# mosaicml/streaming

Measured on AMD Instinct MI355X. Metric: decoded samples/sec + MDS GiB/s, device-resident, at 1/2/4/8 MI355X, higher is better.
Workload: dtype u8

## Files before the change

### streaming_amd/csrc/mdsx_decode.h

```cpp
#pragma once

#include <hip/hip_runtime.h>

#include <cstdint>

#include "mdsx_device.h"
#include "mdsx_internal.h"

namespace mdsx_kernels {

constexpr int kBlock = 256;
constexpr int kSmallMax = 16;
constexpr uint64_t kMapGrain = uint64_t(kBlock) * 16;
constexpr int kGatherRows = 1024;
constexpr int kGroupUnroll = 2;

struct DevCol {
  void* data;
  int64_t* offsets;
  uint8_t* flags;
  uint64_t capacity;
  uint32_t row_bytes;
  int8_t kind;
  int8_t var_index;
  int8_t gather;
  int8_t group;
};

struct TileRun {
  uint64_t stream;
  uint64_t offs;
  uint64_t row0;
  uint32_t bytes;
  uint32_t shard;
  uint32_t r0;
  uint16_t nrows;
  uint16_t fast;
  uint64_t shard_off;
};
static_assert(sizeof(TileRun) == 48, "TileRun layout");

constexpr uint32_t kXcdSeg = 1, kXcdRegister = 2, kXcdRows = 4;

struct DevArgs {
  const uint8_t* batch;
  const mdsx_shard_desc* shards;
  const uint32_t* tile_shard;
  mdsx_status* status;
  int64_t* tile_total;
  int64_t* tile_prefix;
  int64_t* chunk_sum;
  TileRun* tile_run;
  int64_t* totals;
  uint64_t* src_abs;
  uint32_t* row_map;
  uint64_t* lookback;
  uint32_t* ticket;
  uint64_t map_len;
  uint64_t rows;
  uint32_t ntiles;
  uint32_t nscan;
  uint32_t nchunk;
  uint32_t scan_per;
  int32_t nshards;
  int32_t ncols;
  int32_t nvar;
  int32_t tile_rows;
  int16_t any_group;
  int16_t any_wave_str;
  int16_t any_wave_ragged;
  int16_t str_cached;
  uint32_t stage_debug;
  uint32_t run_slots;
  uint32_t rows_bytes;
  uint32_t seg_lim;
  uint32_t seg_small;
  uint32_t xcd_order;
  uint32_t rows_pipe;
  uint32_t rw_k;
  uint32_t swave;
  uint4* sw_rec;
  uint32_t sw_lds;
  uint32_t gather_block0[MDSX_MAX_COLUMNS + 1];
  DevCol cols[MDSX_MAX_COLUMNS];
};


constexpr uint32_t kSwIdle = 0xffffffffu, kSwBad = 0xfffffffeu;

struct TileView {
  const uint8_t* shard;
  const uint32_t* offs;
  mdsx_shard_desc d;
  uint32_t shard_idx;
  uint32_t r0;
  uint32_t nrows;
  uint64_t hdr_end;
  bool table_ok;
};

__device__ __forceinline__ uint32_t xcd_block(uint32_t b, uint32_t n) {
  const uint32_t per = n >> 3;
  return b < per * 8u ? (b & 7u) * per + (b >> 3) : b;
}

__device__ __forceinline__ TileView tile_view(const DevArgs& a, uint32_t tile) {
  TileView v;
  v.shard_idx = a.tile_shard[tile];
  v.d = a.shards[v.shard_idx];
  v.shard = a.batch + v.d.offset;
  v.offs = reinterpret_cast<const uint32_t*>(v.shard + 4);
  v.r0 = (tile - v.d.tile0) * uint32_t(a.tile_rows);
  v.nrows = v.d.samples > v.r0 ? min(uint32_t(a.tile_rows), v.d.samples - v.r0) : 0u;
  v.hdr_end = 4ull + 4ull * (uint64_t(v.d.samples) + 1ull);
  v.table_ok = v.hdr_end <= v.d.bytes;
  return v;
}

__device__ __forceinline__ int sample_range(const TileView& v, uint32_t i, uint32_t* b,
                                            uint32_t* e) {
  *b = v.offs[i];
  *e = v.offs[i + 1];
  if (!(v.hdr_end <= *b && *b <= *e && *e <= v.d.bytes)) return MDSX_E_BOUNDS;
  if (*b == *e) return MDSX_E_EMPTY;
  return MDSX_OK;
}

__device__ __forceinline__ void lds_barrier() {
  asm volatile("s_waitcnt lgkmcnt(0)\n\ts_barrier" ::: "memory");
}

template <bool kRaw = false>
__device__ __forceinline__ int64_t block_exclusive_scan(int64_t x, int64_t* s_wsum,
                                                        int64_t* total) {
  const int lane = threadIdx.x & 63, w = threadIdx.x >> 6;
  int64_t incl = x;
#pragma unroll
  for (int o = 1; o < 64; o <<= 1) {
    const int64_t y = __shfl_up(incl, o);
    if (lane >= o) incl += y;
  }
  if (lane == 63) s_wsum[w] = incl;
  if constexpr (kRaw) lds_barrier();
  else __syncthreads();
  int64_t base = 0, tot = 0;
#pragma unroll
  for (int k = 0; k < kBlock / 64; ++k) {
    const int64_t s = s_wsum[k];
    base += (k < w) ? s : 0;
    tot += s;
  }
  if constexpr (kRaw) lds_barrier();
  else __syncthreads();
  *total = tot;
  return base + incl - x;
}


constexpr uint64_t kHugeCountOffset = 192;
constexpr uint64_t kErrKindsOffset = 64;
constexpr uint32_t kRowLevelErrors = (1u << -MDSX_E_BOUNDS) | (1u << -MDSX_E_EMPTY);

__device__ __forceinline__ void report_decode(const DevArgs& a, int code, int shard, int row,
                                              int col) {
  report(a.status, code, shard, row, col);
  atomicOr(reinterpret_cast<uint32_t*>(reinterpret_cast<uint8_t*>(a.status) + kErrKindsOffset),
           1u << ((-code) & 31));
}

constexpr uint64_t kStatusBlock = 256;

constexpr uint64_t kLbAggregate = 1ull << 62, kLbInclusive = 2ull << 62;
constexpr uint64_t kLbValue = (1ull << 62) - 1;
typedef __attribute__((address_space(1))) uint64_t gu64;

__device__ __forceinline__ void lookback_bases(const DevArgs& a, uint32_t tile, const int64_t* agg,
                                               int64_t* base_out, uint32_t shard, int lane,
                                               uint64_t* words, uint32_t nunits) {
  const int nv = a.nvar;
  const int W = nv <= 1 ? 64 : nv <= 2 ? 32 : nv <= 4 ? 16 : 8;
  const int kk = lane & (W - 1);
  const int seg0 = lane & ~(W - 1);
  const uint64_t wmask = W == 64 ? ~0ull : (1ull << W) - 1;
  for (int g0 = 0; g0 < nv; g0 += 64 / W) {
    const int vi = g0 + lane / W;
    const bool mine = vi < nv;
    gu64* st = (gu64*)(words + uint64_t(mine ? vi : 0) * nunits);
    const uint64_t ag = mine ? uint64_t(agg[vi]) : 0;
    if (mine && kk == 0)
      __hip_atomic_store(st + tile, (tile == 0 ? kLbInclusive : kLbAggregate) | ag,
                         __ATOMIC_RELAXED, __HIP_MEMORY_SCOPE_AGENT);
    uint64_t base = 0;
    int64_t j = int64_t(tile) - 1;
    bool done = !mine || tile == 0;
    uint32_t polls = 0;
    while (__ballot(!done) != 0) {
      const int64_t k = j - kk;
      const uint64_t w = (!done && k >= 0) ? __hip_atomic_load(st + k, __ATOMIC_RELAXED,
                                                               __HIP_MEMORY_SCOPE_AGENT)
                                           : kLbInclusive;
      const uint64_t incl = (__ballot((w >> 62) == 2) >> seg0) & wmask;
      const uint64_t none = (__ballot((w >> 62) == 0) >> seg0) & wmask;
      const uint64_t span = incl ? ((incl & (0 - incl)) << 1) - 1 : wmask;
      const bool wait = !done && (none & span) != 0 && ++polls < (1u << 22);
      uint64_t x = (!done && !wait && ((span >> kk) & 1)) ? (w & kLbValue) : 0;
      for (int o = W >> 1; o > 0; o >>= 1) x += __shfl_xor(x, o);
      if (!done && !wait) {
        if ((none & span) != 0 && kk == 0) report_decode(a, MDSX_E_HIP, int(shard), -1, -1);
        base += x;
        if (incl) done = true;
        else j -= W;
      }
      if (__ballot(wait) != 0) __builtin_amdgcn_s_sleep(1);
    }
    if (mine && kk == 0) {
      if (tile != 0)
        __hip_atomic_store(st + tile, kLbInclusive | (base + ag), __ATOMIC_RELAXED,
                           __HIP_MEMORY_SCOPE_AGENT);
      base_out[vi] = int64_t(base);
      if (tile + 1 == nunits) {
        for (int c = 0; c < a.ncols; ++c)
          if (a.cols[c].var_index == vi) a.cols[c].offsets[a.rows] = int64_t(base + ag);
        if (a.totals) a.totals[vi] = int64_t(base + ag);
      }
    }
  }
}

__device__ __forceinline__ uint32_t draw_ticket(const DevArgs& a, uint32_t* s_tile) {
  if (threadIdx.x == 0) *s_tile = atomicAdd(a.ticket, 1u);
  __syncthreads();
  return __builtin_amdgcn_readfirstlane(*s_tile);
}

int launch_stage_totals(const DevArgs& a, bool nt, hipStream_t s);
int launch_run_decode(const mdsx_plan* plan, const DevArgs& a, hipStream_t s);
int launch_rows_decode(const mdsx_plan* plan, const DevArgs& a, hipStream_t s);
int launch_huge_rows(const DevArgs& a, bool nt, hipStream_t s);
int launch_swave_decode(const mdsx_plan* plan, const DevArgs& a, hipStream_t s);

}
```

### streaming_amd/csrc/mdsx_kernels.hip

```cpp
#include <hip/hip_runtime.h>

#include <algorithm>
#include <cstdint>
#include <cstring>

#include "mdsx_decode.h"
#include "mdsx_device.h"
#include "mdsx_internal.h"

namespace mdsx_kernels {

template <bool kRec = false>
__global__ __launch_bounds__(kBlock) void scan_tiles_kernel(const DevArgs a) {
  __shared__ int64_t s_wsum[kBlock / 64];
  const int t = threadIdx.x;
  const int TR = a.tile_rows;
  const int per_block = kBlock / TR;
  const uint32_t tile = blockIdx.x * uint32_t(per_block) + uint32_t(t / TR);
  const int tt = t % TR;
  const bool tile_ok = tile < a.ntiles;
  TileView v;
  if (tile_ok) v = tile_view(a, tile);
  const uint32_t i = tile_ok ? v.r0 + tt : 0;
  const bool in_tile = tile_ok && v.table_ok && tt < int(v.nrows);
// ... 443 lines not shown
  const int64_t* off;
  const uint64_t* src;
  __device__ __forceinline__ int64_t o(int i) const { return off[i]; }
  __device__ __forceinline__ uint64_t s(int i) const { return src[i]; }
};

template <class Rows>
__device__ __forceinline__ int find_row(const Rows& R, int n, int64_t D) {
  int lo = 0, hi = n - 1;
  while (lo < hi) {
    const int mid = (lo + hi + 1) >> 1;
    if (R.o(mid) <= D) lo = mid; else hi = mid - 1;
  }
  return lo;
}

template <bool kNT, class Rows>
__device__ __forceinline__ uint4 assemble(const Rows& R, int n, int j, int64_t D,
                                          const uint8_t* batch) {
  uint4 acc = make_uint4(0, 0, 0, 0);
  for (; j < n && R.o(j) < D + 16; ++j) {
    const int64_t ro = R.o(j), re = R.o(j + 1);
    const int64_t a = max(D, ro), b = min(D + 16, re);
    if (b <= a) continue;
    const uint64_t s0 = reinterpret_cast<uint64_t>(batch) + R.s(j) + uint64_t(D - ro);
    const uint4* al = reinterpret_cast<const uint4*>(s0 & ~uint64_t(15));
    const uint32_t sh = uint32_t(s0 & 15);
    const uint4 lo = ld16<kNT>(al);
    const uint4 hi = sh ? ld16<kNT>(al + 1) : make_uint4(0, 0, 0, 0);
    const uint4 val = sh ? funnel16_lane(lo, hi, sh) : lo;
    const uint4 m = byte_mask(uint32_t(a - D), uint32_t(b - D));
    acc = make_uint4((acc.x & ~m.x) | (val.x & m.x), (acc.y & ~m.y) | (val.y & m.y),
                     (acc.z & ~m.z) | (val.z & m.z), (acc.w & ~m.w) | (val.w & m.w));
  }
  return acc;
}

template <class Rows>
__device__ __forceinline__ void utf8_check(const Rows& R, int n, int j, int64_t D, int64_t tot,
                                           const uint4 v, uint32_t pw, uint8_t* flags,
                                           uint64_t row0) {
  uint32_t p1 = (pw >> 24) & 0xffu, p2 = (pw >> 16) & 0xffu, p3 = (pw >> 8) & 0xffu;
  const bool ascii = ((v.x | v.y | v.z | v.w) & 0x80808080u) == 0;
  if (ascii && p1 < 0xC0u && p2 < 0xE0u && p3 < 0xF0u) return;
  const int64_t dist = D - R.o(j);
  if (dist < 3) p3 = 0;
  if (dist < 2) p2 = 0;
  if (dist < 1) p1 = 0;
  int64_t rend = R.o(j + 1);
  bool bad = false;
#pragma unroll
  for (int k = 0; k < 16; ++k) {
    const int64_t P = D + k;
    if (P >= tot) break;
    if (P >= rend) {
      if (bad) flags[row0 + j] = 1;
      bad = false;
      do {
        ++j;
        rend = R.o(j + 1);
      } while (P >= rend && j + 1 < n);
      p1 = p2 = p3 = 0;
    }
    const uint32_t b = byte_of(v, k);
    const bool cont = (b & 0xC0u) == 0x80u;
    const bool need = p1 >= 0xC0u || p2 >= 0xE0u || p3 >= 0xF0u;
    const int64_t left = rend - P;
    bad |= cont != need;
    bad |= b == 0xC0u || b == 0xC1u || b >= 0xF5u;
    bad |= (p1 == 0xE0u && b < 0xA0u) || (p1 == 0xEDu && b > 0x9Fu) ||
           (p1 == 0xF0u && b < 0x90u) || (p1 == 0xF4u && b > 0x8Fu);
    bad |= (b >= 0xC0u && left <= 1) || (b >= 0xE0u && left <= 2) || (b >= 0xF0u && left <= 3);
    p3 = p2;
    p2 = p1;
    p1 = b;
  }
  if (bad) flags[row0 + j] = 1;
}

template <bool kNT, int kGatherChunks, class Rows>
__device__ __forceinline__ void gather_tile(const DevArgs& a, const DevCol& col, const Rows& R,
                                            int n, uint64_t r0, int64_t T0, int64_t tot,
                                            uint32_t* s_edge) {
  const bool utf8 = col.kind == MDSX_KIND_STR && col.flags;
  uint8_t* out = static_cast<uint8_t*>(col.data);
  const int lane = threadIdx.x & 63, wave = threadIdx.x >> 6;
  const uint64_t base = reinterpret_cast<uint64_t>(a.batch);
  uint4 val[kGatherChunks], lo[kGatherChunks], hi[kGatherChunks];
  int jrow[kGatherChunks];
  uint32_t shift[kGatherChunks];
  bool single[kGatherChunks], need_hi[kGatherChunks];
#pragma unroll
  for (int k = 0; k < kGatherChunks; ++k) {
    const int64_t D = T0 + 16 * (threadIdx.x + kBlock * k);
    const bool valid = D < tot;
    const int j = valid ? find_row(R, n, D) : 0;
    const int64_t ro = R.o(j), re = R.o(j + 1);
    const uint64_t s0 = base + R.s(j) + uint64_t(D - ro);
    const uint4* al = reinterpret_cast<const uint4*>(s0 & ~uint64_t(15));
    jrow[k] = j;
    shift[k] = uint32_t(s0 & 15);
    single[k] = valid && D + 16 <= re;
    const bool next_same = single[k] && D + 16 < re && lane != 63;
    need_hi[k] = single[k] && shift[k] != 0 && !next_same;
    lo[k] = valid ? ld16<kNT>(al) : make_uint4(0, 0, 0, 0);
    hi[k] = need_hi[k] ? ld16<kNT>(al + 1) : make_uint4(0, 0, 0, 0);
  }
#pragma unroll
  for (int k = 0; k < kGatherChunks; ++k) {
    const int64_t D = T0 + 16 * (threadIdx.x + kBlock * k);
    const uint4 nb = shfl_down1(lo[k]);
    if (single[k]) {
      const uint4 h = need_hi[k] ? hi[k] : nb;
      val[k] = shift[k] ? funnel16_lane(lo[k], h, shift[k]) : lo[k];
    } else if (D < tot) {
      val[k] = assemble<kNT>(R, n, jrow[k], D, a.batch);
    } else {
      val[k] = make_uint4(0, 0, 0, 0);
    }
    if (D < tot) {
      const uint64_t dst = reinterpret_cast<uint64_t>(out) + uint64_t(D);
      if (uint64_t(D) + 16 <= col.capacity) {
        st16<kNT>(dst, val[k]);
      } else {
        for (int b = 0; b < 16 && uint64_t(D) + b < col.capacity; ++b)
          out[D + b] = uint8_t(byte_of(val[k], b));
      }
    }
  }
  if (!utf8) return;
#pragma unroll
  for (int k = 0; k < kGatherChunks; ++k)
    if (lane == 63) s_edge[k * (kBlock / 64) + wave] = val[k].w;
  __syncthreads();
#pragma unroll
  for (int k = 0; k < kGatherChunks; ++k) {
    const int c = threadIdx.x + kBlock * k;
    const int64_t D = T0 + 16 * c;
    uint32_t pw = __shfl_up(val[k].w, 1);
    if (lane == 0) {
      if (c == 0)
        pw = D > R.o(0) ? assemble<kNT>(R, 1, 0, D - 16, a.batch).w : 0u;
      else
        pw = s_edge[wave > 0 ? k * (kBlock / 64) + wave - 1 : (k - 1) * (kBlock / 64) + 3];
    }
    if (D < tot) utf8_check(R, n, jrow[k], D, tot, val[k], pw, col.flags, r0);
  }
}

template <bool kNT, int kGatherChunks>
__global__ __launch_bounds__(kBlock) void gather_ragged_kernel(const DevArgs a) {
  constexpr uint64_t kGatherTile = kMapGrain * kGatherChunks;
  __shared__ __attribute__((aligned(16))) int64_t s_off[kGatherRows + 1];
  __shared__ uint64_t s_src[kGatherRows];
  __shared__ uint32_t s_edge[kGatherChunks * (kBlock / 64)];
  int vi = 0;
  while (vi + 1 < a.nvar && blockIdx.x >= a.gather_block0[vi + 1]) ++vi;
  int ci = 0;
  while (a.cols[ci].var_index != vi) ++ci;
  const DevCol& col = a.cols[ci];
  const int64_t tot = col.offsets[a.rows];
  const uint32_t kinds =
      *reinterpret_cast<const uint32_t*>(reinterpret_cast<const uint8_t*>(a.status) + kErrKindsOffset);
  if (kinds & ~kRowLevelErrors) return;
  const uint32_t* map = a.row_map + uint64_t(vi) * a.map_len;
  const uint64_t* src = a.src_abs + uint64_t(vi) * a.rows;
  const uint64_t stride = a.gather_block0[vi + 1] - a.gather_block0[vi];
  for (uint64_t g = blockIdx.x - a.gather_block0[vi];; g += stride) {
    const int64_t T0 = int64_t(g * kGatherTile);
    if (T0 >= tot || (g + 1) * kGatherChunks >= a.map_len) return;
    const uint64_t r0 = map[g * kGatherChunks];
    const uint64_t r1 =
        (T0 + int64_t(kGatherTile) < tot) ? uint64_t(map[(g + 1) * kGatherChunks]) : a.rows - 1;
    if (r0 >= a.rows || r1 >= a.rows || r1 < r0) return;
    const int n = int(r1 - r0 + 1);
    __syncthreads();
    if (n <= kGatherRows) {
      for (int i = threadIdx.x; i <= n; i += kBlock) {
        s_off[i] = col.offsets[r0 + i];
        if (i < n) s_src[i] = src[r0 + i];
      }
      __syncthreads();
      gather_tile<kNT, kGatherChunks>(a, col, RowsLds{s_off, s_src}, n, r0, T0, tot, s_edge);
    } else {
      gather_tile<kNT, kGatherChunks>(a, col, RowsGlobal{col.offsets + r0, src + r0}, n, r0,
                                      T0, tot, s_edge);
    }
  }
}

struct Layout {
  uint64_t tile_total, tile_prefix, chunk_sum, tile_run, src_abs, row_map, sw_rec, map_len,
      total;
};

__host__ uint64_t round256(uint64_t x) { return (x + 255) & ~uint64_t(255); }

constexpr uint64_t kTicketOffset = 128;

Layout workspace_layout(const mdsx_plan* plan, const mdsx_batch* b) {
  Layout L;
  const uint64_t nv = uint64_t(plan->nvar);
  L.map_len = b->bytes / kMapGrain + 8;
  L.tile_total = 256;
  L.tile_prefix = L.tile_total + round256(nv * b->ntiles * 8);
  L.chunk_sum = L.tile_prefix + round256(nv * b->ntiles * 8);
  L.tile_run = L.chunk_sum + round256(nv * (b->ntiles / kScanChunk + 1) * 8);
  L.src_abs = L.tile_run + round256(nv ? uint64_t(b->ntiles) * sizeof(TileRun) : 0);
  L.row_map = L.src_abs + round256(nv * b->rows * 8);
  L.sw_rec = L.row_map + round256(nv * L.map_len * 4);
  L.total = L.sw_rec + round256(use_swave_decode(plan, b->bytes, b->rows)
                                    ? uint64_t(b->ntiles) *
                                          uint64_t(b->tile_rows ? b->tile_rows
                                                                : uint32_t(plan->tile_rows)) * 16
                                    : 0);
  return L;
}

int build_args(const mdsx_plan* plan, const mdsx_batch* b, const mdsx_column_out* outs,
               void* d_workspace, uint64_t workspace_bytes, int64_t* d_totals, DevArgs* a,
               const uint64_t* mode_bytes = nullptr) {
  if (!plan || !b || !b->data || !b->shards || !b->tile_shard || !d_workspace ||
      b->nshards <= 0)
    return mdsx::fail(MDSX_E_ARG, "mdsx: null argument or empty batch");
  if (plan->ncols > 0 && !outs) return mdsx::fail(MDSX_E_ARG, "mdsx: outs is NULL");
  const Layout L = workspace_layout(plan, b);
  if (workspace_bytes < L.total)
    return mdsx::fail(MDSX_E_ARG, "mdsx: workspace smaller than mdsx_workspace_bytes()");
  std::memset(a, 0, sizeof(*a));
  a->batch = b->data;
  a->shards = b->shards;
  a->tile_shard = b->tile_shard;
  uint8_t* ws = static_cast<uint8_t*>(d_workspace);
  a->status = reinterpret_cast<mdsx_status*>(ws);
  a->tile_total = reinterpret_cast<int64_t*>(ws + L.tile_total);
  a->tile_prefix = reinterpret_cast<int64_t*>(ws + L.tile_prefix);
  a->chunk_sum = reinterpret_cast<int64_t*>(ws + L.chunk_sum);
  a->tile_run = reinterpret_cast<TileRun*>(ws + L.tile_run);
  a->src_abs = reinterpret_cast<uint64_t*>(ws + L.src_abs);
  a->row_map = reinterpret_cast<uint32_t*>(ws + L.row_map);
  a->sw_rec = reinterpret_cast<uint4*>(ws + L.sw_rec);
  a->lookback = reinterpret_cast<uint64_t*>(ws + L.tile_total);
  a->ticket = reinterpret_cast<uint32_t*>(ws + kTicketOffset);
  a->map_len = L.map_len;
  a->totals = d_totals;
  a->rows = b->rows;
  a->ntiles = b->ntiles;
  const int tr = b->tile_rows ? int(b->tile_rows) : plan->tile_rows;
  if (tr < 1 || tr > kBlock || (tr & (tr - 1)))
    return mdsx::fail(MDSX_E_ARG, "mdsx: batch tile_rows must be a power of two in [1, 256]");
  a->stage_debug = uint32_t(plan->stage_debug);
  a->xcd_order = uint32_t(plan->xcd_order);
  a->rw_k = uint32_t(plan->rowwave_k);
  a->swave = use_swave_decode(plan, b->bytes, b->rows) ? 1u : 0u;
  a->run_slots = use_run_decode(plan, b->bytes, b->rows) && !a->swave ? uint32_t(plan->run_slots)
                                                                      : 0u;
  if (a->run_slots && plan->seg) {
    a->seg_lim = a->run_slots * 1024u - 1024u - 32u;
    for (int c = 0; c < plan->ncols; ++c)
      if (plan->cols[c].kind == MDSX_KIND_FIXED && plan->cols[c].row_bytes <= kSmallMax)
        a->seg_small += uint32_t(plan->cols[c].row_bytes);
  }
  a->rows_bytes = use_rows_decode(plan, b->bytes, b->rows)
                      ? rows_stage_bytes(plan, b->bytes / b->rows, tr)
                      : 0u;
  if (a->rows_bytes && rows_lds_bytes_est(plan, a->rows_bytes, uint64_t(tr)) > 160 * 1024)
    a->rows_bytes = 0;
  a->rows_pipe = a->rows_bytes ? uint32_t(plan->rows_pipe) : 0u;
  if (a->run_slots && tr > 32)
    return mdsx::fail(MDSX_E_ARG, "mdsx: streaming decode tiles hold at most 32 rows");
  a->scan_per = (a->run_slots || a->rows_bytes) ? 1u : uint32_t(kBlock / tr);
  a->nscan = (b->ntiles + a->scan_per - 1) / a->scan_per;
  a->nchunk = (a->nscan + kScanChunk - 1) / kScanChunk;
  a->nshards = b->nshards;
  a->ncols = plan->ncols;
  a->nvar = plan->nvar;
  a->tile_rows = tr;
  uint32_t gblocks = 0;
  const uint64_t tile = kMapGrain * uint64_t(plan->gather_chunks);
  for (int c = 0; c < plan->ncols; ++c) {
    const mdsx::ColumnSpec& s = plan->cols[c];
    DevCol& d = a->cols[c];
    d.data = outs[c].data;
    d.offsets = outs[c].offsets;
    d.flags = outs[c].flags;
    d.capacity = outs[c].capacity;
    d.row_bytes = uint32_t(s.row_bytes);
    d.kind = int8_t(s.kind);
    d.var_index = int8_t(s.var_index);
    const uint64_t expect =
        mode_bytes ? std::min(mode_bytes[c], outs[c].capacity) : outs[c].capacity;
    d.gather = s.kind != MDSX_KIND_FIXED && b->rows > 0 &&
               expect < uint64_t(plan->gather_min) * b->rows;
    d.group = s.kind != MDSX_KIND_FIXED && !d.gather && b->rows > 0 &&
              expect < uint64_t(plan->group_max) * b->rows;
    if (s.kind == MDSX_KIND_FIXED) {
      if (!d.data && b->rows > 0)
        return mdsx::fail(MDSX_E_ARG, "mdsx: null data pointer for a fixed column");
    } else {
      if (!d.offsets || (!d.data && d.capacity > 0))
        return mdsx::fail(MDSX_E_ARG, "mdsx: null offsets/data for a ragged column");
    }
  }
  for (int c = 0; c < plan->ncols; ++c) {
    const DevCol& d = a->cols[c];
    if (d.group) a->any_group = 1;
    if (d.kind != MDSX_KIND_FIXED && !d.gather && !d.group) a->any_wave_ragged = 1;
    if (d.kind == MDSX_KIND_STR && d.flags && !d.gather) a->any_wave_str = 1;
    a->str_cached = int16_t(plan->str_cached);
  }
  for (int v = 0; v < plan->nvar; ++v) {
    a->gather_block0[v] = gblocks;
    for (int c = 0; c < plan->ncols; ++c)
      if (plan->cols[c].var_index == v && a->cols[c].gather) {
        const uint64_t expect =
            mode_bytes ? std::min(mode_bytes[c], outs[c].capacity) : outs[c].capacity;
        gblocks += uint32_t(expect > tile ? (expect + tile - 1) / tile : 1);
      }
  }
  a->gather_block0[plan->nvar] = gblocks;
  return MDSX_OK;
}

int hip_check(hipError_t e, const char* what) {
  if (e == hipSuccess) return MDSX_OK;
  return mdsx::fail(MDSX_E_HIP, std::string(what) + ": " + hipGetErrorString(e));
}

constexpr uint64_t kProbeBlock = 256 * 1024 / 16;
__global__ __launch_bounds__(kBlock) void copy_probe_kernel(const uint4* __restrict__ src,
                                                            uint4* __restrict__ dst, uint64_t n) {
  const uint64_t b0 = uint64_t(blockIdx.x) * kProbeBlock;
  const uint64_t b1 = b0 + kProbeBlock < n ? b0 + kProbeBlock : n;
  for (uint64_t base = b0; base < b1; base += kBlock * 8) {
    uint4 v[8];
#pragma unroll
    for (int u = 0; u < 8; ++u) {
      const uint64_t i = base + u * kBlock + threadIdx.x;
      if (i < b1) v[u] = ld16<true>(src + i);
    }
#pragma unroll
    for (int u = 0; u < 8; ++u) {
      const uint64_t i = base + u * kBlock + threadIdx.x;
      if (i < b1) st16<true>(reinterpret_cast<uint64_t>(dst + i), v[u]);
    }
  }
}

template <int U, bool kNT>
__device__ __forceinline__ void rowwave_columns(const DevArgs& a, const TileView& v, uint32_t b,
                                                uint64_t row, int c, int lane) {
  uint32_t pos = 0;
  for (int j = 0; j < c; ++j) pos += a.cols[j].row_bytes;
  for (; c < a.ncols; ++c) {
    const DevCol& col = a.cols[c];
    if (col.row_bytes > uint32_t(kSmallMax))
      wave_copy<false, U, kNT>(v.shard + b + pos,
                               static_cast<uint8_t*>(col.data) + row * col.row_bytes,
                               col.row_bytes, lane);
    pos += col.row_bytes;
  }
}

template <bool kNT, int kW, int kR = 1, int kOcc = 0, int kX = 0>
__global__ __launch_bounds__(64 * kW, kOcc > 0 ? kOcc : 1) void rowwave_decode_kernel(const DevArgs a) {
  constexpr int U = 4;
  const int lane = threadIdx.x & 63;
  const uint32_t blk =
      (a.xcd_order & kXcdRegister) ? xcd_block(blockIdx.x, gridDim.x) : blockIdx.x;
  const uint32_t w =
      blk * kW + (kW == 1 ? 0u : uint32_t(__builtin_amdgcn_readfirstlane(threadIdx.x >> 6)));
  const uint32_t per = uint32_t(a.tile_rows) / kR;
  const uint32_t tile = w / per, rw0 = (w - tile * per) * kR;
  if (tile >= a.ntiles) return;
  const TileView v = tile_view(a, tile);
  if (!v.table_ok) {
    if (rw0 == 0 && lane == 0 && tile == v.d.tile0)
      report_decode(a, MDSX_E_HEADER, v.shard_idx, -1, -1);
    return;
  }
  if (rw0 == 0 && lane == 0 && tile == v.d.tile0) {
    const uint32_t n = *reinterpret_cast<const uint32_t*>(v.shard);
    if (n != v.d.samples || v.offs[0] < v.hdr_end || v.offs[v.d.samples] > v.d.bytes)
      report_decode(a, MDSX_E_HEADER, v.shard_idx, -1, -1);
  }
  if (rw0 >= v.nrows) return;
  const uint32_t nr = min(uint32_t(kR), v.nrows - rw0);
  const uint32_t i0 = v.r0 + rw0;
  const uint64_t row0 = v.d.row0 + i0;
  const int ncols = a.ncols;
  uint32_t size = 0, coff = 0, rb = 0, coff_l = 0, rb_l = 0;
  int cl = -1;
  for (int c = 0; c < ncols; ++c) {
    const uint32_t b = a.cols[c].row_bytes;
    if (lane == c) coff = size, rb = b;
    if (cl < 0 && b > uint32_t(kSmallMax)) cl = c, coff_l = size, rb_l = b;
    size += b;
  }
  const bool small = !(kX & 4) && lane < ncols && rb <= uint32_t(kSmallMax);
  const uint32_t o0 = (kX & 2) ? uint32_t(v.hdr_end) + a.rw_k
                              : __builtin_amdgcn_readfirstlane(v.offs[0]);
  const bool spec0 = o0 >= v.hdr_end;
  uint32_t obv[kR + 1];
#pragma unroll
  for (int k = 0; k <= kR; ++k)
    obv[k] = (kX & 1) ? o0 + (i0 + uint32_t(k)) * size : k <= int(nr) ? v.offs[i0 + uint32_t(k)] : 0u;
  const uint64_t data_l = cl >= 0 ? reinterpret_cast<uint64_t>(a.cols[cl].data) : 0;
  uint4 o[kR];
  uint4 lo[kR][U];
  uint4 tail[kR];
  bool one[kR];
#pragma unroll
  for (int j = 0; j < kR; ++j) {
    const uint64_t pred = uint64_t(o0) + uint64_t(i0 + j) * size;
    const bool spec = j < int(nr) && spec0 && pred + size <= v.d.bytes;
    o[j] = spec && small ? small_load(v.shard + pred + coff, rb) : make_uint4(0, 0, 0, 0);
    const uint64_t d0 = data_l + (row0 + j) * rb_l, dend = d0 + rb_l;
    const uint64_t dbeg = d0 & ~uint64_t(15);
    const uint32_t nch = uint32_t((((dend + 15) & ~uint64_t(15)) - dbeg) >> 4);
    one[j] = spec && cl >= 0 && nch <= 64u * U;
    const uint64_t sfirst = reinterpret_cast<uint64_t>(v.shard + pred + coff_l) - (d0 - dbeg);
    const uint32_t nload = nch + ((sfirst & 15) ? 1u : 0u);
    const uint4* sal = reinterpret_cast<const uint4*>(sfirst & ~uint64_t(15));
    tail[j] = make_uint4(0, 0, 0, 0);
#pragma unroll
    for (int u = 0; u < U; ++u) {
      const uint32_t k = uint32_t(u) * 64u + uint32_t(lane);
      lo[j][u] = one[j] && k < nload ? ld16<kNT>(sal + k) : make_uint4(0, 0, 0, 0);
    }
    if (one[j] && (sfirst & 15) && lane == 63 && 64u * U < nload) tail[j] = ld16<kNT>(sal + 64u * U);
  }
#pragma unroll
  for (int j = 0; j < kR; ++j) {
    if (j >= int(nr)) break;
    const uint32_t i = i0 + j;
    const uint64_t row = row0 + j;
    const uint64_t pred = uint64_t(o0) + uint64_t(i) * size;
    const uint32_t b = __builtin_amdgcn_readfirstlane(obv[j]);
    const uint32_t e = __builtin_amdgcn_readfirstlane(obv[j + 1]);
    if (spec0 && pred + size <= v.d.bytes && b == pred && e >= b && e - b >= size &&
        e <= v.d.bytes) {
      if (small) small_store(static_cast<uint8_t*>(a.cols[lane].data) + row * rb, o[j], rb);
      int c = cl;
      if (one[j]) {
        const uint64_t d0 = data_l + row * rb_l, dend = d0 + rb_l;
        const uint64_t dbeg = d0 & ~uint64_t(15);
        const uint32_t nch = uint32_t((((dend + 15) & ~uint64_t(15)) - dbeg) >> 4);
        const uint32_t sh = uint32_t((reinterpret_cast<uint64_t>(v.shard + pred + coff_l) -
                                      (d0 - dbeg)) & 15);
#pragma unroll
        for (int u = 0; u < U; ++u) {
          const uint32_t k0 = uint32_t(u) * 64u;
          if (k0 >= nch) break;
          const uint32_t k = k0 + uint32_t(lane);
          uint4 out = lo[j][u];
          if (sh != 0) {
            uint4 hi = shfl_down1(lo[j][u]);
            const uint4 nxt = (u + 1 < U) ? readlane0(lo[j][u + 1 < U ? u + 1 : u]) : tail[j];
            if (lane == 63) hi = nxt;
            out = funnel16(lo[j][u], hi, sh);
          }
          const uint64_t D = dbeg + 16ull * k;
          if (k < nch && D >= d0 && D + 16 <= dend) st16<kNT>(D, out);
          if (k0 == 0 && (dbeg < d0 || dbeg + 16 > dend))
            wave_edge_store(out, 0, dbeg, d0, dend, lane);
          if (nch > 1 && (dend & 15) != 0 && nch - 1 >= k0 && nch - 1 < k0 + 64)
            wave_edge_store(out, int(nch - 1 - k0), dbeg + 16ull * (nch - 1), d0, dend, lane);
        }
        ++c;
      }
      if (c >= 0) rowwave_columns<U, kNT>(a, v, b, row, c, lane);
      continue;
    }
    uint32_t bb = 0, ee = 0;
    int rc = sample_range(v, i, &bb, &ee);
    if (rc == MDSX_OK && uint64_t(bb) + size > ee) rc = MDSX_E_BOUNDS;
    if (rc != MDSX_OK) {
      if (lane == 0) report_decode(a, rc, v.shard_idx, int(i), -1);
      continue;
    }
    if (small)
      gather_small(v.shard + bb + coff, static_cast<uint8_t*>(a.cols[lane].data) + row * rb, rb);
    rowwave_columns<U, kNT>(a, v, bb, row, 0, lane);
  }
}

template <int kU, bool kNTLoad, bool kNTStore, bool kXcd = false, int kWaves = kBlock / 64>
__global__ __launch_bounds__(64 * kWaves) void copy_wave_kernel(const uint4* __restrict__ src,
                                                                uint4* __restrict__ dst,
                                                                uint64_t n) {
  const uint32_t blk = kXcd ? xcd_block(blockIdx.x, gridDim.x) : blockIdx.x;
  const uint64_t w = uint64_t(blk) * kWaves + (threadIdx.x >> 6);
  const uint64_t b0 = w * (64 * kU) + (threadIdx.x & 63);
  uint4 v[kU];
#pragma unroll
  for (int u = 0; u < kU; ++u) {
    const uint64_t i = b0 + 64 * u;
    if (i < n) v[u] = ld16<kNTLoad>(src + i);
  }
#pragma unroll
  for (int u = 0; u < kU; ++u) {
    const uint64_t i = b0 + 64 * u;
    if (i < n) st16<kNTStore>(reinterpret_cast<uint64_t>(dst + i), v[u]);
  }
}



constexpr int kGatherRowTile = 256;

struct OneSrc {
  const uint8_t* vals;
  const int64_t* off;
  const uint8_t* flags;
  uint64_t rows;
  __device__ __forceinline__ bool resolve(int64_t id, mdsx_gather_src* g, uint64_t* r) const {
    if (id < 0 || uint64_t(id) >= rows) return false;
    g->values = vals;
    g->offsets = off;
    g->flags = flags;
    *r = uint64_t(id);
    return true;
  }
};

struct MultiSrc {
  const mdsx_gather_src* table;
  uint32_t n;
  __device__ __forceinline__ bool resolve(int64_t id, mdsx_gather_src* g, uint64_t* r) const {
    const uint64_t s = uint64_t(id) >> MDSX_GATHER_SRC_SHIFT;
    if (id < 0 || s >= n) return false;
    *g = table[s];
    *r = uint64_t(id) & ((uint64_t(1) << MDSX_GATHER_SRC_SHIFT) - 1);
    return *r < g->rows;
  }
};

template <bool kNT, class Src>
__global__ __launch_bounds__(kBlock) void gather_fixed_kernel(const Src S, uint32_t row_bytes,
                                                              const int64_t* idx, uint64_t m,
                                                              uint8_t* dst, mdsx_status* st) {
  const uint64_t k0 = uint64_t(blockIdx.x) * kGatherRowTile;
  const int lane = threadIdx.x & 63, wave = threadIdx.x >> 6;
  if (row_bytes <= uint32_t(kSmallMax)) {
    const uint64_t k = k0 + threadIdx.x;
    if (k < m) {
      mdsx_gather_src g;
      uint64_t r;
      if (!S.resolve(idx[k], &g, &r)) {
        report(st, MDSX_E_BOUNDS, -1, int(k), -1);
      } else {
        const MDSX_G uint8_t* p = gp(static_cast<const uint8_t*>(g.values) + r * row_bytes);
        MDSX_G uint8_t* q = gp(dst + k * row_bytes);
        switch (row_bytes) {
          case 1: *q = *p; break;
          case 2: *(MDSX_G uint16_t*)q = *(const MDSX_G uint16_t*)p; break;
          case 4: *(MDSX_G uint32_t*)q = *(const MDSX_G uint32_t*)p; break;
          case 8: *(MDSX_G uint64_t*)q = *(const MDSX_G uint64_t*)p; break;
          case 16: *(MDSX_G u32x4*)q = *(const MDSX_G u32x4*)p; break;
          default:
            for (uint32_t j = 0; j < row_bytes; ++j) q[j] = p[j];
        }
      }
    }
    return;
  }
  const bool aligned = (row_bytes & 15) == 0;
  for (int i = wave; i < kGatherRowTile; i += kBlock / 64) {
    const uint64_t k = k0 + i;
    if (k >= m) break;
    mdsx_gather_src g;
    uint64_t r;
    if (!S.resolve(idx[k], &g, &r)) {
      if (lane == 0) report(st, MDSX_E_BOUNDS, -1, int(k), -1);
      continue;
    }
    const uint8_t* src = static_cast<const uint8_t*>(g.values) + r * row_bytes;
    if (aligned)
      wave_copy<false, 4, kNT, false>(src, dst + k * row_bytes, row_bytes, lane);
    else
      wave_copy<false, 4, kNT, true, true>(src, dst + k * row_bytes, row_bytes, lane);
  }
}

template <class Src>
__global__ __launch_bounds__(kBlock) void gather_len_kernel(const Src S, const int64_t* idx,
                                                            uint64_t m, int64_t* dst_off,
                                                            int64_t* tile_total, mdsx_status* st) {
  __shared__ int64_t s_wsum[kBlock / 64];
  const uint64_t k = uint64_t(blockIdx.x) * kGatherRowTile + threadIdx.x;
  int64_t len = 0;
  if (k < m) {
    mdsx_gather_src g;
    uint64_t r;
    if (!S.resolve(idx[k], &g, &r))
      report(st, MDSX_E_BOUNDS, -1, int(k), -1);
    else
      len = g.offsets[r + 1] - g.offsets[r];
  }
  int64_t total;
  const int64_t excl = block_exclusive_scan(len, s_wsum, &total);
  if (k < m) dst_off[k] = excl;
  if (threadIdx.x == 0) tile_total[blockIdx.x] = total;
}

__global__ __launch_bounds__(kBlock) void scan_tile_totals_kernel(const int64_t* in, int64_t* out,
                                                                  uint32_t n, int64_t* dst_off,
                                                                  uint64_t m, int64_t* out_total) {
  __shared__ int64_t s_wsum[kBlock / 64];
  int64_t carry = 0;
  for (uint32_t base = 0; base < n; base += kBlock) {
    const uint32_t k = base + threadIdx.x;
    const int64_t x = k < n ? in[k] : 0;
    int64_t total;
    const int64_t excl = block_exclusive_scan(x, s_wsum, &total);
    if (k < n) out[k] = carry + excl;
    carry += total;
  }
  if (threadIdx.x == 0) {
    dst_off[m] = carry;
    if (out_total) *out_total = carry;
  }
}

template <bool kNT, bool kGroup, class Src>
__global__ __launch_bounds__(kBlock) void gather_copy_kernel(
    const Src S, const int64_t* idx, uint64_t m, uint8_t* dst_vals, uint64_t capacity,
    int64_t* dst_off, uint8_t* dst_flags, const int64_t* tile_prefix, mdsx_status* st) {
  __shared__ const uint8_t* s_src[kGatherRowTile];
  __shared__ int64_t s_dst[kGatherRowTile];
  __shared__ int64_t s_len[kGatherRowTile];
  const uint64_t k0 = uint64_t(blockIdx.x) * kGatherRowTile;
  const int lane = threadIdx.x & 63, wave = threadIdx.x >> 6;
  {
    const uint64_t k = k0 + threadIdx.x;
    int64_t len = -1;
    if (k < m) {
      const int64_t off = tile_prefix[blockIdx.x] + dst_off[k];
      dst_off[k] = off;
      s_dst[threadIdx.x] = off;
      mdsx_gather_src g;
      uint64_t r;
      if (S.resolve(idx[k], &g, &r)) {
        s_src[threadIdx.x] = static_cast<const uint8_t*>(g.values) + g.offsets[r];
        len = g.offsets[r + 1] - g.offsets[r];
        if (uint64_t(off + len) > capacity) {
          report(st, MDSX_E_CAPACITY, -1, int(k), -1);
          len = -1;
        }
        if (dst_flags) dst_flags[k] = g.flags ? g.flags[r] : 0;
      }
    }
    s_len[threadIdx.x] = len;
  }
  __syncthreads();
  if constexpr (kGroup) {
    const int g = lane >> 4;
    for (int r0 = wave * 4; r0 < kGatherRowTile; r0 += kBlock / 16) {
      if (k0 + r0 >= m) break;
      const int i = r0 + g;
      const bool live = k0 + i < m && s_len[i] > 0;
      group_copy<2, kNT, true>(live ? s_src[i] : dst_vals, live ? dst_vals + s_dst[i] : dst_vals,
                               live ? uint64_t(s_len[i]) : 0, lane);
    }
  } else {
    for (int i = wave; i < kGatherRowTile; i += kBlock / 64) {
      if (k0 + i >= m) break;
      const int64_t len = s_len[i];
      if (len <= 0) continue;
      wave_copy<false, 4, kNT, true, true>(s_src[i], dst_vals + s_dst[i], uint64_t(len), lane);
    }
  }
}


__device__ __forceinline__ bool value_dtype_ok(uint32_t id) {
  return id == 8 || id == 9 || id == 16 || id == 17 || id == 18 || id == 32 || id == 33 ||
         id == 34 || id == 64 || id == 65 || id == 66;
}

__device__ __forceinline__ uint64_t read_uint(const uint8_t* p, int nbytes) {
  uint64_t v = 0;
  for (int b = 0; b < nbytes; ++b) v |= uint64_t(p[b]) << (8 * b);
  return v;
}

template <bool kShapes>
__global__ __launch_bounds__(kBlock) void ndarray_meta_kernel(
    const uint8_t* values, const int64_t* offsets, uint64_t rows, int dtype_id, uint8_t* out_dtype,
    uint8_t* out_ndim, int64_t* out_data_offset, int64_t* out_numel, uint8_t* out_bad,
    int32_t* max_ndim, int32_t shape_cols, int64_t* out_shape) {
  const uint64_t r = uint64_t(blockIdx.x) * kBlock + threadIdx.x;
  if (r >= rows) return;
  const int64_t b = offsets[r], e = offsets[r + 1];
  const uint8_t* p = values + b;
  const int64_t len = e - b;
  int64_t pos = 0;
  bool bad = false;
  uint32_t id = uint32_t(dtype_id);
  if (id == 0) {
    if (len < 1) bad = true;
    else id = p[pos++];
    if (!bad && !value_dtype_ok(id)) bad = true;
  }
  uint32_t ndim = 0, code = 0;
  if (!bad) {
    if (pos + 1 > len) bad = true;
    else {
      const uint32_t byte = p[pos++];
      ndim = byte >> 2;
      code = byte & 3;
    }
  }
  const int sbytes = 1 << code;
  const int64_t want = int64_t(ndim) * sbytes;
  if (!bad && want > len - pos) {
    if ((len - pos) % sbytes) bad = true;
    else ndim = uint32_t((len - pos) / sbytes);
  }
  const int64_t item = int64_t(id >> 3);
  int64_t prod = item;
  bool zero = false;
  if (!bad) {
    for (uint32_t k = 0; k < ndim; ++k) {
      const uint64_t dim = read_uint(p + pos + k * sbytes, sbytes);
      if (kShapes && int32_t(k) < shape_cols) out_shape[r * shape_cols + k] = int64_t(dim);
      if (dim > uint64_t(INT64_MAX)) { bad = true; break; }
      if (dim == 0) { zero = true; continue; }
      if (__builtin_mul_overflow(prod, int64_t(dim), &prod)) { bad = true; break; }
    }
    pos = pos + want < len ? pos + want : len;
  }
  const int64_t numel = (bad || zero) ? 0 : prod / item;
  if (!bad && (len - pos) != numel * item) bad = true;
  if (kShapes) {
    for (int32_t k = int32_t(ndim); k < shape_cols; ++k) out_shape[r * shape_cols + k] = 1;
    return;
  }
  out_dtype[r] = uint8_t(bad ? 0 : id);
  out_ndim[r] = uint8_t(bad ? 0 : ndim);
  out_data_offset[r] = b + pos;
  out_numel[r] = bad ? 0 : numel;
  out_bad[r] = bad ? 1 : 0;
  if (!bad && max_ndim) atomicMax(max_ndim, int32_t(ndim));
}
// ... 558 lines not shown
```

Baseline: 768.0 million.

## Precompute row layout on host and use scalar loads in row-wise decode

Moves the per-launch column offset/size scan into host-side setup (new rw_size, rw_cl, col_off fields), so the kernel no longer loops over columns per wave. Offset-table reads now go through a constant address space pointer so they become scalar loads, and column parameters are forced into SGPRs. The small-column load is split into raw word loads with alignment applied at store time, and the shard header check moves after the loads are issued so it stops blocking them. This aims to cut per-wave scalar/vector instruction overhead and load latency, at the cost of larger kernel args and reliance on scalar-load assumptions about uniform offsets.

```diff
diff --git a/streaming_amd/csrc/mdsx_decode.h b/streaming_amd/csrc/mdsx_decode.h
--- a/streaming_amd/csrc/mdsx_decode.h
+++ b/streaming_amd/csrc/mdsx_decode.h
@@ -39,6 +39,17 @@
   uint64_t shard_off;
 };
 static_assert(sizeof(TileRun) == 48, "TileRun layout");
+
+#define MDSX_K __attribute__((address_space(4)))
+template <class T>
+__device__ __forceinline__ const MDSX_K T* kp(const T* p) {
+  return (const MDSX_K T*)p;
+}
+template <class T>
+__device__ __forceinline__ T sgpr(T x) {
+  asm volatile("" : "+s"(x));
+  return x;
+}
 
 constexpr uint32_t kXcdSeg = 1, kXcdRegister = 2, kXcdRows = 4;
 
@@ -81,6 +92,11 @@
   uint32_t swave;
   uint4* sw_rec;
   uint32_t sw_lds;
+  uint32_t rw_size;
+  uint32_t rw_coff_l;
+  uint32_t rw_rb_l;
+  int32_t rw_cl;
+  uint32_t col_off[MDSX_MAX_COLUMNS];
   uint32_t gather_block0[MDSX_MAX_COLUMNS + 1];
   DevCol cols[MDSX_MAX_COLUMNS];
 };
diff --git a/streaming_amd/csrc/mdsx_kernels.hip b/streaming_amd/csrc/mdsx_kernels.hip
--- a/streaming_amd/csrc/mdsx_kernels.hip
+++ b/streaming_amd/csrc/mdsx_kernels.hip
@@ -769,6 +769,13 @@
         return mdsx::fail(MDSX_E_ARG, "mdsx: null offsets/data for a ragged column");
     }
   }
+  a->rw_cl = -1;
+  for (int c = 0; c < plan->ncols; ++c) {
+    const uint32_t rb = a->cols[c].row_bytes;
+    a->col_off[c] = a->rw_size;
+    if (a->rw_cl < 0 && rb > uint32_t(kSmallMax)) a->rw_cl = c, a->rw_coff_l = a->rw_size, a->rw_rb_l = rb;
+    a->rw_size += rb;
+  }
   for (int c = 0; c < plan->ncols; ++c) {
     const DevCol& d = a->cols[c];
     if (d.group) a->any_group = 1;
@@ -827,6 +834,25 @@
                                col.row_bytes, lane);
     pos += col.row_bytes;
   }
+}
+
+struct SmallRaw {
+  uint32_t w[5];
+  uint32_t r;
+  __device__ __forceinline__ uint4 aligned() const {
+    return make_uint4(alignbyte(w[1], w[0], r), alignbyte(w[2], w[1], r), alignbyte(w[3], w[2], r),
+                      alignbyte(w[4], w[3], r));
+  }
+};
+__device__ __forceinline__ SmallRaw small_load_raw(const uint8_t* p, uint32_t size, bool on) {
+  const uint64_t a = reinterpret_cast<uint64_t>(p);
+  const MDSX_G uint32_t* q = gp_at<const uint32_t>(a & ~uint64_t(3));
+  const uint32_t nd = on ? (size + 6) >> 2 : 0u;
+  SmallRaw s;
+  s.r = uint32_t(a & 3);
+#pragma unroll
+  for (int k = 0; k < 5; ++k) s.w[k] = nd > uint32_t(k) ? q[k] : 0u;
+  return s;
 }
 
 template <bool kNT, int kW, int kR = 1, int kOcc = 0, int kX = 0>
@@ -846,34 +872,37 @@
       report_decode(a, MDSX_E_HEADER, v.shard_idx, -1, -1);
     return;
   }
-  if (rw0 == 0 && lane == 0 && tile == v.d.tile0) {
-    const uint32_t n = *reinterpret_cast<const uint32_t*>(v.shard);
-    if (n != v.d.samples || v.offs[0] < v.hdr_end || v.offs[v.d.samples] > v.d.bytes)
-      report_decode(a, MDSX_E_HEADER, v.shard_idx, -1, -1);
-  }
-  if (rw0 >= v.nrows) return;
-  const uint32_t nr = min(uint32_t(kR), v.nrows - rw0);
+  if (rw0 >= v.nrows && !(rw0 == 0 && tile == v.d.tile0)) return;
+  const uint32_t nr = rw0 < v.nrows ? min(uint32_t(kR), v.nrows - rw0) : 0u;
   const uint32_t i0 = v.r0 + rw0;
   const uint64_t row0 = v.d.row0 + i0;
   const int ncols = a.ncols;
-  uint32_t size = 0, coff = 0, rb = 0, coff_l = 0, rb_l = 0;
-  int cl = -1;
-  for (int c = 0; c < ncols; ++c) {
-    const uint32_t b = a.cols[c].row_bytes;
-    if (lane == c) coff = size, rb = b;
-    if (cl < 0 && b > uint32_t(kSmallMax)) cl = c, coff_l = size, rb_l = b;
-    size += b;
+  const uint32_t size = a.rw_size, coff_l = a.rw_coff_l, rb_l = a.rw_rb_l;
+  const int cl = a.rw_cl;
+  uint32_t coff = 0, rb = 0;
+  for (int c0 = 0; c0 < ncols; c0 += 4) {
+    uint32_t co[4], cb[4];
+#pragma unroll
+    for (int k = 0; k < 4; ++k)
+      co[k] = sgpr(a.col_off[c0 + k]), cb[k] = sgpr(a.cols[c0 + k].row_bytes);
+#pragma unroll
+    for (int k = 0; k < 4; ++k) {
+      const bool mine = lane == c0 + k;
+      coff = mine ? co[k] : coff;
+      rb = mine ? cb[k] : rb;
+    }
   }
   const bool small = !(kX & 4) && lane < ncols && rb <= uint32_t(kSmallMax);
-  const uint32_t o0 = (kX & 2) ? uint32_t(v.hdr_end) + a.rw_k
-                              : __builtin_amdgcn_readfirstlane(v.offs[0]);
+  const MDSX_K uint32_t* const koffs = kp(v.offs);
+  const uint32_t o0 = (kX & 2) ? uint32_t(v.hdr_end) + a.rw_k : koffs[0];
   const bool spec0 = o0 >= v.hdr_end;
   uint32_t obv[kR + 1];
 #pragma unroll
   for (int k = 0; k <= kR; ++k)
-    obv[k] = (kX & 1) ? o0 + (i0 + uint32_t(k)) * size : k <= int(nr) ? v.offs[i0 + uint32_t(k)] : 0u;
+    obv[k] = (kX & 1) ? o0 + (i0 + uint32_t(k)) * size
+                      : nr > 0 && k <= int(nr) ? koffs[i0 + uint32_t(k)] : 0u;
   const uint64_t data_l = cl >= 0 ? reinterpret_cast<uint64_t>(a.cols[cl].data) : 0;
-  uint4 o[kR];
+  SmallRaw sr[kR];
   uint4 lo[kR][U];
   uint4 tail[kR];
   bool one[kR];
@@ -881,7 +910,7 @@
   for (int j = 0; j < kR; ++j) {
     const uint64_t pred = uint64_t(o0) + uint64_t(i0 + j) * size;
     const bool spec = j < int(nr) && spec0 && pred + size <= v.d.bytes;
-    o[j] = spec && small ? small_load(v.shard + pred + coff, rb) : make_uint4(0, 0, 0, 0);
+    sr[j] = small_load_raw(v.shard + pred + coff, rb, spec && small);
     const uint64_t d0 = data_l + (row0 + j) * rb_l, dend = d0 + rb_l;
     const uint64_t dbeg = d0 & ~uint64_t(15);
     const uint32_t nch = uint32_t((((dend + 15) & ~uint64_t(15)) - dbeg) >> 4);
@@ -897,17 +926,23 @@
     }
     if (one[j] && (sfirst & 15) && lane == 63 && 64u * U < nload) tail[j] = ld16<kNT>(sal + 64u * U);
   }
+  __builtin_amdgcn_sched_barrier(0);
+  if (rw0 == 0 && lane == 0 && tile == v.d.tile0) {
+    const uint32_t n = *reinterpret_cast<const uint32_t*>(v.shard);
+    if (n != v.d.samples || v.offs[0] < v.hdr_end || v.offs[v.d.samples] > v.d.bytes)
+      report_decode(a, MDSX_E_HEADER, v.shard_idx, -1, -1);
+  }
 #pragma unroll
   for (int j = 0; j < kR; ++j) {
     if (j >= int(nr)) break;
     const uint32_t i = i0 + j;
     const uint64_t row = row0 + j;
     const uint64_t pred = uint64_t(o0) + uint64_t(i) * size;
-    const uint32_t b = __builtin_amdgcn_readfirstlane(obv[j]);
-    const uint32_t e = __builtin_amdgcn_readfirstlane(obv[j + 1]);
+    const uint32_t b = obv[j], e = obv[j + 1];
     if (spec0 && pred + size <= v.d.bytes && b == pred && e >= b && e - b >= size &&
         e <= v.d.bytes) {
-      if (small) small_store(static_cast<uint8_t*>(a.cols[lane].data) + row * rb, o[j], rb);
+      if (small)
+        small_store(static_cast<uint8_t*>(a.cols[lane].data) + row * rb, sr[j].aligned(), rb);
       int c = cl;
       if (one[j]) {
         const uint64_t d0 = data_l + row * rb_l, dend = d0 + rb_l;
```

Measured after the change: 785.2 million, median of 6. 2.2% higher.
